# Bismarrck/tensoralloy

Hardware: AMD Instinct MI355X
Metric: atom-steps/sec (energy+forces), 4000-atom Ni rcut=6.5 A (higher is better)
Workload: dtype f64

## Files before the change

tensoralloy_amd/csrc/ta_api.hip:

```cpp
#include <hip/hip_runtime.h>

#include <algorithm>
#include <chrono>
#include <climits>
#include <cmath>
#include <cstdio>
#include <cstdlib>
#include <cstring>
#include <stdexcept>
#include <string>
#include <vector>

#include "ta_device.h"
#include "ta_internal.h"
#include "ta_md.h"

namespace ta {
size_t mlp_scratch_doubles(const MlpDev &mlp);
void launch_mlp_impl(const MlpDev &mlp, int activation, int ndim, const int32_t *atoms, int n_atoms,
                     const DeviceBatch &b, double *scratch, hipStream_t s, MlpLaunchInfo *info = nullptr);
size_t mlp_all_scratch_doubles(const MlpDev *mlps_host, int nel, const int32_t *elem_start);
size_t td_scratch_doubles(const MlpDev *nets, int nel, int K, const int32_t *elem_start);
void launch_td_all(const MlpDev *nets_dev, const MlpDev *nets_host, int nel, int K, int act_h, int act,
                   int sommerfeld, int ndim, const DeviceBatch &b, const double *T, double *u_atom,
// ... 1974 lines not shown
  if (h->kind != TA_MODEL_SF_MLP || !h->sf.angular)
    return fail(h, TA_ERR_INVALID, "only symmetry-function models with angular terms have triples");
  return guarded(h, [&]() {
    compute_impl(h, TA_WANT_ENERGY, false, nullptr);
    h->nl_stats.ensure(8);
    hipStream_t s = h->stream;
    HIP_CHECK(hipMemsetAsync(h->nl_stats.ptr, 0, sizeof(unsigned long long), s));
    const int64_t N = h->db.n_atoms;
    if (N)
      hipLaunchKernelGGL(count_triples_kernel, dim3((unsigned)((N * 64 + 255) / 256)), dim3(256), 0, s, h->db,
                         h->sf.acut * h->sf.acut, h->sf.eps, h->nl_stats.ptr, 1);
    HIP_CHECK(hipGetLastError());
    unsigned long long v = 0;
    HIP_CHECK(hipMemcpyAsync(&v, h->nl_stats.ptr, sizeof(v), hipMemcpyDeviceToHost, s));
    HIP_CHECK(hipStreamSynchronize(s));
    *n_owned = (int64_t)v;
  });
}

int ta_set_triangles(ta_handle h, int on) {
  if (!h) return TA_ERR_INVALID;
  h->triangles = on != 0;
  return TA_OK;
}

int ta_backward_variant(ta_handle h, int32_t *variant) {
  if (!h || !variant) return fail(h, TA_ERR_INVALID, "null argument");
  *variant = h->last_bwd_variant;
  return TA_OK;
}

int ta_mlp_launch_info(ta_handle h, int64_t *info) {
  if (!h || !info) return fail(h, TA_ERR_INVALID, "null argument");
  const ta::MlpLaunchInfo &m = h->last_mlp_launch;
  info[0] = m.family;
  info[1] = m.threads;
  info[2] = m.lh;
  info[3] = m.nt;
  info[4] = m.grid_x;
  info[5] = m.grid_y;
  info[6] = m.lds_bytes;
  info[7] = m.da;
  return TA_OK;
}

int ta_triangle_owner(int64_t n, const int32_t *abc, int32_t *owner) {
  if (n < 0 || (n > 0 && (!abc || !owner))) return TA_ERR_INVALID;
  for (int64_t t = 0; t < n; ++t) {
    int32_t a = abc[3 * t], b = abc[3 * t + 1], c = abc[3 * t + 2];
    if (a > b) std::swap(a, b);
    if (b > c) std::swap(b, c);
    if (a > b) std::swap(a, b);
    const int32_t sorted[3] = {a, b, c};
    owner[t] = (a == b || b == c) ? -1 : sorted[ta::triangle_owner_rank((uint32_t)a + (uint32_t)b + (uint32_t)c)];
  }
  return TA_OK;
}

int ta_measure_hbm_copy(ta_handle h, int64_t bytes, int32_t reps, double *gbs) {
  if (!h || !gbs || bytes < 16 || reps < 1) return fail(h, TA_ERR_INVALID, "bad argument");
  return guarded(h, [&]() {
    const size_t n = (size_t)bytes / 16;
    double2 *src = nullptr, *dst = nullptr;
    HIP_CHECK(hipMalloc((void **)&src, n * 16));
    if (hipMalloc((void **)&dst, n * 16) != hipSuccess) {
      (void)hipFree(src);
      throw std::bad_alloc();
    }
    hipStream_t s = h->stream;
    hipEvent_t e0, e1;
    HIP_CHECK(hipEventCreate(&e0));
    HIP_CHECK(hipEventCreate(&e1));
    HIP_CHECK(hipMemsetAsync(src, 0, n * 16, s));
    static const int per_cu = std::getenv("TA_COPY_WG_PER_CU") ? std::atoi(std::getenv("TA_COPY_WG_PER_CU")) : 8;
    const unsigned blocks = (unsigned)std::min<size_t>((n + 255) / 256, (size_t)256 * std::max(1, per_cu));
    static const int only = std::getenv("TA_COPY_MODE") ? std::atoi(std::getenv("TA_COPY_MODE")) : -1;
    double best = 0.0;
    for (int mode = 0; mode < 3; ++mode) {
      if (only >= 0 && mode != only) continue;
      auto one = [&]() {
        if (mode == 1) (void)hipMemcpyAsync(dst, src, n * 16, hipMemcpyDeviceToDevice, s);
        else if (mode == 2) hipLaunchKernelGGL(hbm_copy_nt_kernel, dim3(blocks), dim3(256), 0, s, src, dst, n);
        else hipLaunchKernelGGL(hbm_copy_kernel, dim3(blocks), dim3(256), 0, s, src, dst, n);
      };
      for (int k = 0; k < 2; ++k) one();
      HIP_CHECK(hipEventRecord(e0, s));
      for (int k = 0; k < reps; ++k) one();
      HIP_CHECK(hipEventRecord(e1, s));
      HIP_CHECK(hipEventSynchronize(e1));
      float ms = 0.f;
      HIP_CHECK(hipEventElapsedTime(&ms, e0, e1));
      if (ms > 0.f) best = std::max(best, 2.0 * (double)(n * 16) * reps / (ms * 1e-3) / 1e9);
    }
    (void)hipEventDestroy(e0);
    (void)hipEventDestroy(e1);
    (void)hipFree(src);
    (void)hipFree(dst);
    *gbs = best;
  });
}

int ta_set_stream(ta_handle h, void *stream) {
  if (!h) return TA_ERR_INVALID;
  return guarded(h, [&]() {
    HIP_CHECK(hipStreamSynchronize(h->stream));
    h->upload_pending = false;
    h->stream = stream ? (hipStream_t)stream : h->own_stream;
// ... 835 lines not shown
```

tensoralloy_amd/csrc/ta_device.h:

```cpp
#pragma once
#include <hip/hip_runtime.h>

#include <cstdint>

#include "tensoralloy_amd.h"

namespace ta {

constexpr int kMaxRadial = 64;
constexpr int kMaxElements = 8;
constexpr int kMaxBetaSlots = 3;
constexpr int kRecDoubles = 8;
constexpr int kMaxLayers = 8;
constexpr int kCapMin = 192;
constexpr int kCapMax = 1024;
constexpr int kMaxCentersPerBlock = 16;
constexpr int kMaxHd = 24;

struct SFParams {
  double rcut, acut;
  double inv_rc2, inv_ac2;
  double two_inv_ac2;
  double eps;
  double ang_scale;
// ... 20 lines not shown
  int chan[8];
  int safe_pow;
  int n_hd;
  double hd[kMaxHd];
};

struct DeviceBatch {
  int64_t n_atoms = 0, n_pairs = 0;
  int n_frames = 0, nnl_max = 0;
  double *pos = nullptr;
  double *cells = nullptr;
  int32_t *species = nullptr;
  int32_t *frame_of_atom = nullptr;
  int32_t *atom_start = nullptr;
  int32_t *pair_start = nullptr;
  int32_t *pair_stop = nullptr;
  int32_t *seg_start = nullptr;
  int32_t *pair_i = nullptr, *pair_j = nullptr, *pair_shift = nullptr, *pair_rev = nullptr;
  const int32_t *slot_q = nullptr, *rev_super = nullptr, *rev_map = nullptr;
  int32_t *blk_center = nullptr;
  int n_blk = 0;
  int blk_groups = 0;
  const int32_t *n_blk_dev = nullptr;
  int cap = kCapMin;
  int32_t *elem_atoms = nullptr;
  int32_t elem_start[kMaxElements + 1] = {0};

  double *rec = nullptr;
  double *rec4 = nullptr;
  double *part4 = nullptr;
  unsigned long long *masks = nullptr;
  uint32_t *job_word = nullptr;
  int32_t *job_count = nullptr;
  int job_stride = 0;
  uint32_t *job_word_own = nullptr;
  int32_t *job_count_own = nullptr;
  double *G = nullptr;
  double *dEdG = nullptr;
  double *eatom = nullptr;
  double *g = nullptr;
  double *forces = nullptr;
  double *wat = nullptr;
  double *fown = nullptr;
  int own_sums = 0;
#ifdef TA_PHASE_STAMPS
  unsigned long long *stamps = nullptr;
#endif
  double *bpart = nullptr;
  double *energy = nullptr;
  double *virial = nullptr;
  double *batch_energy = nullptr;
};

__host__ __device__ inline int triangle_owner_rank(uint32_t index_sum) {
#ifdef __HIP_DEVICE_COMPILE__
  const uint32_t h = __umul24(index_sum, 0x9E3779u);
#else
  const uint32_t h = index_sum * 0x9E3779u;
#endif
  return (int)(((h & 0xFFFFFFu) * 3u) >> 24);
}
__host__ __device__ inline bool owns_triangle(int32_t i, int32_t j, int32_t k) {
  return triangle_owner_rank((uint32_t)i + (uint32_t)j + (uint32_t)k) == (j < i ? 1 : 0) + (k < i ? 1 : 0);
}

#ifdef __HIPCC__
__device__ __forceinline__ int pair_stop_of(const DeviceBatch &b, int64_t i) {
  return b.pair_stop ? b.pair_stop[i] : b.pair_start[i + 1];
}
#endif

#ifdef __HIPCC__
__device__ __forceinline__ int pair_rev_of(const DeviceBatch &b, int q) {
  return b.slot_q ? b.rev_map[b.rev_super[b.slot_q[q]]] : b.pair_rev[q];
}
__device__ __forceinline__ const double2 *pair_geom(const DeviceBatch &b, size_t q) {
  return reinterpret_cast<const double2 *>(b.rec4 ? b.rec4 + 4 * q : b.rec + kRecDoubles * q);
}
#endif

struct MlpLayerDev {
  int k, n;
  int kp, np;
  double *w;
  double *wt;
  double *b;
  int act;
  int res;
};
struct MlpDev {
  int n_layers = 0;
  MlpLayerDev layer[kMaxLayers];
  double *xlo = nullptr, *xhi = nullptr;
  int max_np = 0, max_kp = 0;
};

struct MlpLaunchInfo {
  int family = 0;
  int threads = 0;
  int lh = 0;
  int nt = 0;
  int grid_x = 0, grid_y = 0;
  long long lds_bytes = 0;
  int da = 0;
};

void launch_pair_geometry(const SFParams &sf, const DeviceBatch &b, hipStream_t s);
void launch_g4_forward(const SFParams &sf, const AngChunk &ch, int nb, int ng, int nz,
                       const DeviceBatch &b, hipStream_t s);
void launch_descriptor_reduce(const SFParams &sf, const DeviceBatch &b, hipStream_t s);
void launch_mlp(const SFParams &sf, const MlpDev &mlp, int activation, int element,
                const DeviceBatch &b, hipStream_t s);
void launch_backward(const SFParams &sf, const AngChunk &ch, int nb, int ng, int nz,
                     bool first, bool radial_only, const DeviceBatch &b, hipStream_t s);
void launch_force_gather(const SFParams &sf, const DeviceBatch &b, hipStream_t s);
void launch_frame_reduce(const DeviceBatch &b, bool want_virial, double *mirror, int64_t n_tail, hipStream_t s);
// ... 68 lines not shown
```

tensoralloy_amd/csrc/ta_kernels_v2.hip:

```cpp
#include <hip/hip_runtime.h>

#include <cstdio>
#include <cstdlib>
#include <stdexcept>
#include <type_traits>

#include "ta_device.h"
#include "ta_math.h"
#include "ta_reduce.h"

namespace ta {
namespace {

constexpr int kBlock = 256;
constexpr int kNF = 8;
constexpr int kNFf = 7;
constexpr int kSegW = 6;
constexpr int kOwnCtl = 60 + 2 * kMaxCentersPerBlock * kSegW;
constexpr int kJobCtlBytes = (kOwnCtl + 40) * 4;
__host__ __device__ inline int v2_pcols(int cap, int nspec) {
  return nspec >= 1 ? cap / 4 + kMaxCentersPerBlock * nspec : cap;
}
constexpr int kRingPad = 64;
constexpr int kRTab = 8;

#ifdef TA_LDS_PROBE
__device__ __forceinline__ bool kProbe(int flags, int bit) { return (flags >> bit) & 1; }
#else
__device__ __forceinline__ constexpr bool kProbe(int, int) { return false; }
#endif

#ifdef TA_PHASE_STAMPS
#define TA_STAMP(b, kernel, k)                                                                          \
  do {                                                                                                  \
    if ((b).stamps && threadIdx.x == 0)                                                                 \
      (b).stamps[((size_t)(kernel) * gridDim.x + blockIdx.x) * 8 + (k)] = __builtin_amdgcn_s_memrealtime(); \
  } while (0)
#else
#define TA_STAMP(b, kernel, k) do {} while (0)
#endif

__device__ __forceinline__ int angular_term2(int s1, int s2, int nel) {
  int a = s1 < s2 ? s1 : s2, b = s1 < s2 ? s2 : s1;
  return a * nel - (a * (a - 1)) / 2 + (b - a);
}
__device__ __forceinline__ int radial_term2(int center, int other) {
  return other == center ? 0 : (other < center ? other + 1 : other);
}

struct Fields {
  double2 *zr, *xy, *ih, *gs;
  double *sp1;
  float *xf, *yf, *zf;
};

__device__ __forceinline__ Fields carve(double *lds, int cap, bool forward = false) {
  Fields f;
  f.zr = reinterpret_cast<double2 *>(lds);
  f.xy = f.zr + cap;
  f.ih = f.xy + cap;
  f.gs = forward ? nullptr : f.ih + cap;
  f.sp1 = forward ? reinterpret_cast<double *>(f.ih + cap) : nullptr;
  f.xf = forward ? reinterpret_cast<float *>(f.sp1 + cap) : nullptr;
  f.yf = forward ? f.xf + (2 * cap + kRingPad) : nullptr;
  f.zf = forward ? f.yf + (2 * cap + kRingPad) : nullptr;
  return f;
}

template <int HD>
__device__ __forceinline__ void hd_eval(const SFParams &sf, const AngChunk &ch, double beta,
                                        double u, double &h, double &dh) {
  if constexpr (HD > 0) {
    double p = ch.hd[HD - 1], d = 0.0;
#pragma unroll
    for (int k = HD - 2; k >= 0; --k) {
      d = fma(d, u, p);
      p = fma(p, u, ch.hd[k]);
    }
    h = p;
    dh = d;
  } else {
    double fd, dfd;
    cutoff_u(sf.cutoff, u, fd, dfd);
    const double ed = ta_exp(-beta * u);
    h = ed * fd;
    dh = ed * (dfd - beta * fd);
  }
}
template <int HD>
__device__ __forceinline__ double hd_value(const SFParams &sf, const AngChunk &ch, double beta,
                                           double u) {
  if constexpr (HD > 0) {
    double p = ch.hd[HD - 1];
#pragma unroll
    for (int k = HD - 2; k >= 0; --k) p = fma(p, u, ch.hd[k]);
    return p;
  } else {
    return ta_exp(-beta * u) * cutoff_u_value(sf.cutoff, u);
  }
}

template <int HD>
__device__ __forceinline__ void stage(const SFParams &sf, const AngChunk &ch, double beta, const DeviceBatch &b,
                                      const Fields &f, int s0, int M, int geom = 0, bool forward = false,
                                      int *jidx = nullptr) {
  for (int item = threadIdx.x; item < M; item += blockDim.x) {
    double2 v0, v1, v2;
    if (geom) {
      const int64_t p = (int64_t)s0 + item;
      const int i = b.pair_i[p], j = b.pair_j[p];
      const double *h = b.cells + 9 * (size_t)b.frame_of_atom[i];
      const double sx = (double)b.pair_shift[3 * p], sy = (double)b.pair_shift[3 * p + 1],
                   sz = (double)b.pair_shift[3 * p + 2];
      const double *ri = b.pos + 3 * (size_t)i, *rj = b.pos + 3 * (size_t)j;
      const double dx = (rj[0] - ri[0]) + (sx * h[0] + sy * h[3] + sz * h[6]);
      const double dy = (rj[1] - ri[1]) + (sx * h[1] + sy * h[4] + sz * h[7]);
      const double dz = (rj[2] - ri[2]) + (sx * h[2] + sy * h[5] + sz * h[8]);
      const double r2 = dx * dx + dy * dy + dz * dz + sf.eps;
      v0 = make_double2(dx, dy);
      v1 = make_double2(dz, r2);
      v2 = make_double2(1.0 / sqrt(r2), 0.0);
      if (b.rec4) {
        double2 *dst = reinterpret_cast<double2 *>(b.rec4 + 4 * (size_t)p);
        dst[0] = v0;
        dst[1] = v1;
      } else {
        double2 *dst = reinterpret_cast<double2 *>(b.rec + kRecDoubles * (size_t)p);
        dst[0] = v0;
        dst[1] = v1;
        dst[2] = v2;
        dst[3] = make_double2(0.0, 0.0);
      }
    } else if (b.rec4) {
      const double2 *src = reinterpret_cast<const double2 *>(b.rec4 + 4 * (size_t)(s0 + item));
      v0 = src[0];
      v1 = src[1];
      v2 = make_double2(1.0 / sqrt(v1.y), 0.0);
    } else {
      const double2 *src = reinterpret_cast<const double2 *>(b.rec + kRecDoubles * (size_t)(s0 + item));
      v0 = src[0];
      v1 = src[1];
      v2 = src[2];
    }
    f.xy[item] = v0;
    f.zr[item] = v1;
    if (forward) {
      const int ci = b.pair_i[s0 + item];
      const int cbase = b.pair_start[ci] - s0, cn = pair_stop_of(b, ci) - b.pair_start[ci];
      const int k0 = 2 * cbase + (item - cbase);
      f.xf[k0] = f.xf[k0 + cn] = (float)v0.x;
      f.yf[k0] = f.yf[k0 + cn] = (float)v0.y;
      f.zf[k0] = f.zf[k0 + cn] = (float)v1.x;
    }
    const double u = v1.y * sf.inv_ac2;
    double H = 0.0, L = 0.0;
    if (u < 1.0) {
      if (forward) {
        H = hd_value<HD>(sf, ch, beta, u);
      } else {
        double dH;
        hd_eval<HD>(sf, ch, beta, u, H, dH);
        L = (H != 0.0) ? sf.two_inv_ac2 * dH / H : 0.0;
      }
    }
    f.ih[item] = make_double2(v2.x, H);
    if (jidx) jidx[item] = b.pair_j[s0 + item];
    else if (forward) f.sp1[item] = (double)b.species[b.pair_j[s0 + item]];
    else f.gs[item] = make_double2(L, (double)b.species[b.pair_j[s0 + item]]);
  }
  __syncthreads();
}

__device__ __forceinline__ unsigned long long partner_mask(const SFParams &sf, const Fields &f,
                                                           int base, int n, int a, int sc, int smax) {
  const int ring = 2 * base + a;
  const float ax = f.xf[ring], ay = f.yf[ring], az = f.zf[ring];
  const float lim = (float)(sf.acut * sf.acut) * 1.0001f;
  unsigned long long mask = 0ull;
  const int count = smax - sc + 1;
  typedef float f32x2 __attribute__((ext_vector_type(2)));
  const f32x2 ax2 = {ax, ax}, ay2 = {ay, ay}, az2 = {az, az};
  for (int g = 0; g < 4 && 16 * g < count; ++g) {
    const float *px = f.xf + ring + sc + 16 * g, *py = f.yf + ring + sc + 16 * g,
                *pz = f.zf + ring + sc + 16 * g;
    unsigned m = 0u;
#pragma unroll
    for (int k = 14; k >= 0; k -= 2) {
      const f32x2 vx = {px[k], px[k + 1]}, vy = {py[k], py[k + 1]}, vz = {pz[k], pz[k + 1]};
      const f32x2 ex = vx - ax2, ey = vy - ay2, ez = vz - az2;
      const f32x2 d2 = __builtin_elementwise_fma(ex, ex, __builtin_elementwise_fma(ey, ey, ez * ez));
      const float dhi = d2.y, dlo = d2.x;
      asm("v_cmp_lt_f32 vcc, %1, %2\n\tv_addc_co_u32 %0, vcc, %0, %0, vcc" : "+v"(m) : "v"(dhi), "v"(lim) : "vcc");
      asm("v_cmp_lt_f32 vcc, %1, %2\n\tv_addc_co_u32 %0, vcc, %0, %0, vcc" : "+v"(m) : "v"(dlo), "v"(lim) : "vcc");
    }
    mask |= (unsigned long long)m << (16 * g);
  }
  if (count < 64) mask &= (1ull << count) - 1ull;
  const int half = n >> 1;
  if (!(n & 1) && a >= half && half >= sc && half < sc + 64) mask &= ~(1ull << (half - sc));
  return mask;
}

__device__ __forceinline__ void deal_by_popcount(const Fields &f, int cap, int M, int &item,
                                                 unsigned long long &mask) {
  int *hist = reinterpret_cast<int *>(f.xf);
  int *start = hist + 66;
  unsigned long long *pmask = reinterpret_cast<unsigned long long *>(hist + 132);
  int *pitem = reinterpret_cast<int *>(pmask + cap);
  const int tid = threadIdx.x;
  const bool active = tid < M;
  __syncthreads();
  if (tid < 66) hist[tid] = 0;
  __syncthreads();
  const int bucket = 64 - (active ? __popcll(mask) : 0);
  int rank = 0;
  if (active) rank = atomicAdd(&hist[bucket], 1);
  __syncthreads();
  if (tid < 65) {
    int s = 0;
// ... 68 lines not shown
  }
  const int n = j.start[16];
  __syncthreads();
  return n;
}

__device__ __forceinline__ int job_slot(int r, int tid, int T) { return r * T + ((r & 1) ? T - 1 - tid : tid); }

__device__ __forceinline__ void make_owned_jobs(int *hist, int *start, const uint32_t word[4], const unsigned own[4],
                                                uint32_t *out, int32_t *count) {
  const int tid = threadIdx.x;
  int cnt[4], rank[4] = {0, 0, 0, 0};
#pragma unroll
  for (int r = 0; r < 4; ++r) {
    cnt[r] = __popc(own[r]);
    if (cnt[r]) rank[r] = atomicAdd(&hist[16 - cnt[r]], 1);
  }
  __syncthreads();
  if (tid < 64) {
    const int v = tid < 16 ? hist[tid] : 0;
    int incl = v;
#pragma unroll
    for (int off = 1; off < 16; off <<= 1) {
      const int u = __shfl_up(incl, off);
      if (tid >= off) incl += u;
    }
    if (tid < 16) start[tid] = incl - v;
    if (tid == 15) *count = incl;
  }
  __syncthreads();
#pragma unroll
  for (int r = 0; r < 4; ++r)
    if (cnt[r]) out[start[16 - cnt[r]] + rank[r]] = (word[r] & 0xffffu) | (own[r] << 16);
}

template <int NG, int NZ>
__device__ __forceinline__ void defz_coeffs(const AngChunk &ch, const double *wsrc, double pc[5]) {
  double p0 = 0.0, p1 = 0.0, p2 = 0.0, p3 = 0.0, p4 = 0.0;
#pragma unroll
  for (int ig = 0; ig < NG; ++ig) {
    const double g1 = ch.gamma[ig], g2 = g1 * g1;
    const double w1 = wsrc[ch.chan[ig * NZ]] * ch.kz[0], w4 = wsrc[ch.chan[ig * NZ + 1]] * ch.kz[1];
    p0 += w1 + w4;
    p1 += g1 * (w1 + 4.0 * w4);
    p2 += 6.0 * g2 * w4;
    p3 += 4.0 * g2 * g1 * w4;
    p4 += g2 * g2 * w4;
  }
  pc[0] = p0;
  pc[1] = 0.5 * p1;
  pc[2] = 0.25 * p2;
  pc[3] = 0.125 * p3;
  pc[4] = 0.0625 * p4;
}

__device__ __forceinline__ double rsqrt_f64(double x) {
  double y = __builtin_amdgcn_rsq(x);
  const double hx = 0.5 * x;
  y = fma(y, fma(-hx * y, y, 0.5), y);
  y = fma(y, fma(-hx * y, y, 0.5), y);
  return y;
}

__device__ __forceinline__ void reduce_radial_from_lds(const SFParams &sf, const DeviceBatch &b,
                                                       const Fields &f, int c0, int c1, int s0) {
  const int nel = sf.n_elements;
  const int w = threadIdx.x >> 6, l = threadIdx.x & 63, nwaves = blockDim.x >> 6;
  bool no_shift = true;
  for (int c = 0; c < sf.n_rad; ++c) no_shift = no_shift && sf.omega[c] == 0.0;
  for (int64_t i = c0 + w; i < c1; i += nwaves) {
    const int sA = b.species[i];
    const int32_t *seg = b.seg_start + (size_t)i * (nel + 1);
    double *Gi = b.G + (size_t)i * sf.ndim;
    for (int sb = 0; sb < nel; ++sb) {
      const int tr = radial_term2(sA, sb);
      const int q0 = seg[sb] - s0, q1 = seg[sb + 1] - s0;
      for (int cc = 0; cc < sf.n_rad; cc += 4) {
        double acc[4] = {0.0, 0.0, 0.0, 0.0};
        for (int q = q0 + l; q < q1; q += 64) {
          const double r2 = f.zr[q].y;
          const double u = r2 * sf.inv_rc2;
          const double fc = (u < 1.0) ? cutoff_u_value(sf.cutoff, u) : 0.0;
          if (no_shift) {
#pragma unroll
            for (int k = 0; k < 4; ++k) {
              const int c = (cc + k < sf.n_rad) ? cc + k : cc;
              acc[k] += ta_exp(-sf.eta[c] * u) * fc;
            }
          } else {
            const double r = sqrt(r2);
#pragma unroll
            for (int k = 0; k < 4; ++k) {
              const int c = (cc + k < sf.n_rad) ? cc + k : cc;
              const double dr = r - sf.omega[c];
              acc[k] += ta_exp(-sf.eta[c] * dr * dr * sf.inv_rc2) * fc;
            }
          }
        }
#pragma unroll
        for (int k = 0; k < 4; ++k) {
          const double v = wave_sum(acc[k]);
          if (l == 0 && cc + k < sf.n_rad) Gi[tr * sf.n_rad + cc + k] = v;
        }
      }
    }
  }
// ... 89 lines not shown
        const int *ss = sslot + ci * kSegW;
        const double *colA = P + (size_t)(sa * kGZ + gz) * v2_pcols(cap, NSPEC);
        for (int q = ss[sb] + l; q < ss[sb + 1]; q += 16) v += colA[q];
        if (sa != sb) {
          const double *colB = P + (size_t)(sb * kGZ + gz) * v2_pcols(cap, NSPEC);
          for (int q = ss[sa] + l; q < ss[sa + 1]; q += 16) v += colB[q];
        }
        v = row16_sum(v);
        if (l == 0) Gi[sf.n_radial_dim + term * sf.n_ang + ch.chan[gz]] = v * sf.ang_scale;
      }
    }
  }
}

__device__ __forceinline__ void stagger(int flags) {
  const int n = (flags >> 8) & 0xff;
  if (n && ((blockIdx.x >> ((flags >> 16) & 31)) & 1))
    for (int k = 0; k < n; ++k) __builtin_amdgcn_s_sleep(127);
}

template <int NSPEC, int NG, int NZ, int HD, bool DEFZ, int CAP, int WPE = (DEFZ && NSPEC <= 2 ? 5 : 0)>
__global__ __launch_bounds__(kBlock)
    __attribute__((amdgpu_waves_per_eu(WPE > 0 ? WPE : 1, 8))) void g4_forward_v2_kernel(SFParams sf, AngChunk ch,
                                                               DeviceBatch b, int flags) {
  static_assert(!DEFZ || NZ == 2, "DEFZ needs the two-zeta grid");
  const int kCap = CAP > 0 ? CAP : b.cap;
  const int geom = flags & 1;
  if (b.n_blk_dev && (int)blockIdx.x >= *b.n_blk_dev) return;
  stagger(flags);
  extern __shared__ double lds[];
  const Fields f = carve(lds, kCap, true);
  const int slot = b.blk_groups > 0 ? 16 * ((int)blockIdx.x % b.blk_groups) + (int)blockIdx.x / b.blk_groups
                                    : (int)blockIdx.x;
  const int c0 = b.blk_center[slot], c1 = b.blk_center[slot + 1];
  if (c0 >= c1) return;
  const int s0 = b.pair_start[c0];
  const int M = pair_stop_of(b, c1 - 1) - s0;
  const double beta = ch.beta[0];
  if (b.job_count) {
    char *raw = reinterpret_cast<char *>(lds);
    int *cnt = reinterpret_cast<int *>(raw + v2_counter_offset(kCap));
    if (threadIdx.x < 40) cnt[threadIdx.x] = 0;
    else if (threadIdx.x < 40 + 17 && (int)threadIdx.x - 40 <= c1 - c0)
      cnt[threadIdx.x] = ((int)threadIdx.x - 40 < c1 - c0 ? b.pair_start[c0 + threadIdx.x - 40] : s0 + M) - s0;
    else if (threadIdx.x >= 64 && (int)threadIdx.x - 64 < (c1 - c0) * (NSPEC + 1)) {
      const int k = ((int)threadIdx.x - 64) / (NSPEC + 1), sg = ((int)threadIdx.x - 64) % (NSPEC + 1);
      cnt[60 + k * kSegW + sg] = b.seg_start[(size_t)(c0 + k) * (NSPEC + 1) + sg] - s0;
    }
    if (NSPEC == 1 && b.job_word_own && threadIdx.x < 20) cnt[kOwnCtl + threadIdx.x] = 0;
    double *P0 = reinterpret_cast<double *>(raw + v2_counter_offset(kCap) + kJobCtlBytes);
    for (int k = threadIdx.x; k < NSPEC * NG * NZ * v2_pcols(kCap, NSPEC); k += blockDim.x) P0[k] = 0.0;
  }
  int *jidx = (NSPEC == 1 && b.job_word_own && b.job_count) ? reinterpret_cast<int *>(f.sp1) : nullptr;
  TA_STAMP(b, 0, 0);
  stage<HD>(sf, ch, beta, b, f, s0, M, geom, true, jidx);
  TA_STAMP(b, 0, 1);
  if (b.job_count && threadIdx.x == 0) {
    int *ctl = reinterpret_cast<int *>(reinterpret_cast<char *>(lds) + v2_counter_offset(kCap));
    const int *segl = ctl + 60;
    int *sslot = ctl + 60 + kMaxCentersPerBlock * kSegW;
    int acc = 0;
    for (int k = 0; k < c1 - c0; ++k)
      for (int sg = 0; sg <= NSPEC; ++sg) {
        sslot[k * kSegW + sg] = acc;
        if (sg < NSPEC) acc += (segl[k * kSegW + sg + 1] - segl[k * kSegW + sg] + 3) >> 2;
      }
  }

  auto run_item = [&](int item, bool have_mask, unsigned long long mask0, double *out, double *pacc, auto is_job) {
    constexpr bool kJob = decltype(is_job)::value;
    const int64_t p = (int64_t)s0 + item;
    int base, n;
    int pslot = item;
    unsigned own = 0u;
    int kbit = 0;
    uint32_t sij = 0u;
    int ic = 0, rij = 0;
    if constexpr (kJob) {
      const int *cstart = reinterpret_cast<const int *>(reinterpret_cast<const char *>(lds) + v2_counter_offset(kCap)) + 40;
      const int ci = job_centre((uint32_t)mask0);
      if (NSPEC == 1 && jidx) {
        ic = c0 + ci;
        const int j = jidx[item];
        sij = (uint32_t)ic + (uint32_t)j;
        rij = j < ic ? 1 : 0;
      }
      base = cstart[ci];
      n = cstart[ci + 1] - base;
      {
        const int *segl = cstart + 20, *sslot = segl + kMaxCentersPerBlock * kSegW;
        const int sg = NSPEC == 1 ? 0 : (int)f.sp1[item];
        pslot = sslot[ci * kSegW + sg] + ((item - segl[ci * kSegW + sg]) >> 2);
      }
    } else {
      const int i = b.pair_i[p];
      base = b.pair_start[i] - s0;
      n = pair_stop_of(b, i) - b.pair_start[i];
    }
    const int a = item - base;
    const double2 axy = f.xy[item], azr = f.zr[item], aih = f.ih[item];
    const double ax = axy.x, ay = axy.y, az = azr.x;
    const double ra2 = azr.y, inv_ra = aih.x, Ha = aih.y;

    double acc[NSPEC][NG][NZ];
#pragma unroll
    for (int sp = 0; sp < NSPEC; ++sp)
#pragma unroll
      for (int ig = 0; ig < NG; ++ig)
#pragma unroll
        for (int iz = 0; iz < NZ; ++iz) acc[sp][ig][iz] = 0.0;
    double mom[NSPEC][5];
#pragma unroll
    for (int sp = 0; sp < NSPEC; ++sp)
#pragma unroll
      for (int k = 0; k < 5; ++k) mom[sp][k] = 0.0;

    auto triple = [&](int bl) {
        bl = (int)min((unsigned)bl, (unsigned)bl - (unsigned)n);
        const int q = kProbe(flags, 30) ? (int)threadIdx.x : base + bl;
        const double2 bxy = f.xy[q], bzr = f.zr[q];
        const double ex = bxy.x - ax, ey = bxy.y - ay, ez = bzr.x - az;
        const double d2 = fma(ex, ex, fma(ey, ey, fma(ez, ez, sf.eps)));
        const double u = kProbe(flags, 30) ? 0.5 : d2 * sf.inv_ac2;
        if (!(u < 1.0)) return;
        if constexpr (kJob && NSPEC == 1) {
          if (jidx) {
            const int kk = jidx[q];
            own |= (triangle_owner_rank(sij + (uint32_t)kk) == rij + (kk < ic ? 1 : 0) ? 1u : 0u) << kbit;
          }
        }
        const double2 bih = f.ih[kProbe(flags, 29) ? (int)threadIdx.x : q];
        const double cth = (ra2 + bzr.y - d2) * 0.5 * inv_ra * bih.x;
        const double common = Ha * bih.y * hd_value<HD>(sf, ch, beta, u);
        const int sb = NSPEC == 1 ? 0 : (int)f.sp1[q];
        if constexpr (DEFZ) {
          const double c2 = cth * cth;
          const double t1 = common * cth, t2 = common * c2, t3 = t1 * c2, t4 = t2 * c2;
#pragma unroll
          for (int sp = 0; sp < NSPEC; ++sp) {
            const bool on = NSPEC == 1 || sb == sp;
            mom[sp][0] += on ? common : 0.0;
            mom[sp][1] += on ? t1 : 0.0;
            mom[sp][2] += on ? t2 : 0.0;
            mom[sp][3] += on ? t3 : 0.0;
            mom[sp][4] += on ? t4 : 0.0;
          }
        } else {
#pragma unroll
          for (int ig = 0; ig < NG; ++ig) {
            const double basev = fma(ch.gamma[ig], cth, 1.0);
#pragma unroll
            for (int iz = 0; iz < NZ; ++iz) {
              double pw;
              if (ch.zeta_int[iz] > 0)
                pw = pow_int_m1(basev, ch.zeta_int[iz]) * basev;
              else
                pw = safe_pow_value(ch.safe_pow, basev, ch.zeta[iz]);
              const double v = pw * common;
#pragma unroll
              for (int sp = 0; sp < NSPEC; ++sp)
                acc[sp][ig][iz] += (NSPEC == 1 || sb == sp) ? v : 0.0;
            }
          }
        }
    };
    if constexpr (kJob) {
      const uint32_t jw = (uint32_t)mask0;
      unsigned m = (flags & (1 << 24)) ? 0u : jw >> 16;
      const int k0 = a + 1 + 16 * (int)((jw >> 8) & 3u);
      while (m) {
        const int k = __ffs((int)m) - 1;
        m &= m - 1;
        kbit = k;
        triple(k0 + k);
      }
    } else {
    const int smax = (Ha != 0.0) ? n / 2 : 0;
    for (int sc = 1; sc <= smax; sc += 64) {
      unsigned long long mask;
      if (have_mask) {
        mask = (flags & (1 << 24)) ? 0ull : mask0;
      } else {
        mask = partner_mask(sf, f, base, n, a, sc, smax);
        if (b.masks) b.masks[(size_t)(sc >> 6) * b.n_pairs + p] = mask;
      }
      while (mask) {
        const int k = __ffsll((long long)mask) - 1;
        mask &= mask - 1;
        triple(a + sc + k);
      }
    }
    }
    if constexpr (DEFZ) {
#pragma unroll
      for (int sp = 0; sp < NSPEC; ++sp)
#pragma unroll
        for (int ig = 0; ig < NG; ++ig) {
          const double g1 = ch.gamma[ig], g2 = g1 * g1;
          acc[sp][ig][0] = fma(g1, mom[sp][1], mom[sp][0]);
          acc[sp][ig][1] = fma(g2 * g2, mom[sp][4], fma(4.0 * g2 * g1, mom[sp][3],
                               fma(6.0 * g2, mom[sp][2], fma(4.0 * g1, mom[sp][1], mom[sp][0]))));
        }
    }
#pragma unroll
    for (int sp = 0; sp < NSPEC; ++sp)
#pragma unroll
      for (int ig = 0; ig < NG; ++ig)
#pragma unroll
        for (int iz = 0; iz < NZ; ++iz) {
          const int c = ch.chan[ig * NZ + iz];
          const double v = acc[sp][ig][iz] * ch.kz[iz];
          if (pacc) {
            if (v != 0.0) atomicAdd(&pacc[(size_t)((sp * NG + ig) * NZ + iz) * v2_pcols(kCap, NSPEC) + pslot], v);
          } else if (out)
            out[(sp * NG + ig) * NZ + iz] = v;
          else
            b.part4[(size_t)(sp * sf.n_ang + c) * b.n_pairs + p] = v;
        }
    return own;
  };

  int item = threadIdx.x;
  const bool active = item < M;
  int n_own = 0;
  if (active) {
    const int i = b.pair_i[s0 + item];
    n_own = pair_stop_of(b, i) - b.pair_start[i];
  }
  const bool one_pass = M <= (int)blockDim.x && !__syncthreads_or(active && (n_own >> 1) > 64);
  if (one_pass) {
    unsigned long long mask = 0ull;
    if (active) {
      const int64_t p = (int64_t)s0 + item;
      const int i = b.pair_i[p];
      const int base = b.pair_start[i] - s0;
      const int smax = (f.ih[item].y != 0.0) ? n_own / 2 : 0;
      if (smax > 0 && !(flags & (1 << 25))) mask = partner_mask(sf, f, base, n_own, item - base, 1, smax);
      if (b.masks && !b.job_count) b.masks[p] = mask;
    }
    TA_STAMP(b, 0, 2);
    if (b.job_count) {
      char *raw = reinterpret_cast<char *>(lds);
      JobLists jl = job_lists(f);
      jl.hist = reinterpret_cast<int *>(raw + v2_counter_offset(kCap));
      jl.start = jl.hist + 20;
      double *P = reinterpret_cast<double *>(raw + v2_counter_offset(kCap) + kJobCtlBytes);
      const int n_jobs = make_jobs(jl, active, item, active ? b.pair_i[s0 + item] - c0 : 0, mask);
      TA_STAMP(b, 0, 3);
      const size_t jbase = (size_t)blockIdx.x * b.job_stride;
      if (threadIdx.x == 0) b.job_count[blockIdx.x] = n_jobs;
      for (int slot = threadIdx.x; slot < n_jobs; slot += blockDim.x) b.job_word[jbase + slot] = jl.word[slot];
      TA_STAMP(b, 0, 4);
      uint32_t swept[4] = {0u, 0u, 0u, 0u};
      unsigned owned[4] = {0u, 0u, 0u, 0u};
      if (!(flags & (1 << 27)))
        for (int r = 0; r * (int)blockDim.x < n_jobs; ++r) {
          const int slot = job_slot(r, threadIdx.x, blockDim.x);
          if (slot < n_jobs) {
            const uint32_t jw = jl.word[slot];
            const unsigned o = run_item(job_item(jw), true, jw, nullptr, P, std::true_type{});
            if (r < 4) {
              swept[r] = jw;
              owned[r] = o;
            }
          }
        }
      if (jidx)
        make_owned_jobs(jl.hist + kOwnCtl, jl.hist + kOwnCtl + 20, swept, owned, b.job_word_own + jbase,
                        b.job_count_own + blockIdx.x);
      __syncthreads();
      TA_STAMP(b, 0, 5);
      if (flags & 4) {
        assemble_flat<NSPEC, NG, NZ>(sf, ch, b, f, P, jl.hist + 60 + kMaxCentersPerBlock * kSegW, c0, c1, s0, item, active,
                                     (flags & (1 << 26)) != 0, kCap);
        TA_STAMP(b, 0, 6);
        return;
      }
      if (active) {
        const int64_t p = (int64_t)s0 + threadIdx.x;
        const int ci = b.pair_i[p] - c0, sg = NSPEC == 1 ? 0 : (int)f.sp1[threadIdx.x];
        const int *segl = jl.hist + 60, *sslot = segl + kMaxCentersPerBlock * kSegW;
        const int rel = (int)threadIdx.x - segl[ci * kSegW + sg];
        const int pidx = sslot[ci * kSegW + sg] + (rel >> 2);
        const bool holds = (rel & 3) == 0;
#pragma unroll
        for (int sp = 0; sp < NSPEC; ++sp)
#pragma unroll
          for (int gz = 0; gz < NG * NZ; ++gz)
            b.part4[(size_t)(sp * sf.n_ang + ch.chan[gz]) * b.n_pairs + p] =
                holds ? P[(size_t)(sp * NG * NZ + gz) * v2_pcols(kCap, NSPEC) + pidx] : 0.0;
      }
    } else {
    deal_by_popcount(f, kCap, M, item, mask);
    constexpr int kLocal = NSPEC * NG * NZ;
    constexpr int kGZ = NG * NZ;
    constexpr int kSpPerPass = 8 / kGZ;
    if (flags & 4) {
      double mine[kLocal];
#pragma unroll
      for (int k = 0; k < kLocal; ++k) mine[k] = 0.0;
      if (active) run_item(item, true, mask, mine, nullptr, std::false_type{});
      __syncthreads();
      double *red = reinterpret_cast<double *>(f.xy);
#pragma unroll
      for (int sp_lo = 0; sp_lo < NSPEC; sp_lo += kSpPerPass) {
        const int sp_hi = sp_lo + kSpPerPass < NSPEC ? sp_lo + kSpPerPass : NSPEC;
        if (active) {
#pragma unroll
          for (int k = 0; k < kSpPerPass * kGZ; ++k)
            if (sp_lo * kGZ + k < kLocal) red[(size_t)k * kCap + item] = mine[sp_lo * kGZ + k];
        }
        __syncthreads();
        if (sp_lo == 0) reduce_radial_from_lds(sf, b, f, c0, c1, s0);
        reduce_angular_from_lds<NSPEC, NG, NZ>(sf, ch, b, red, kCap, c0, c1, s0, sp_lo, sp_hi);
        __syncthreads();
      }
      return;
    }
    if (active) run_item(item, true, mask, nullptr, nullptr, std::false_type{});
    }
  } else {
    if (b.job_count && threadIdx.x == 0) b.job_count[blockIdx.x] = -1;
    if (jidx && threadIdx.x == 0) b.job_count_own[blockIdx.x] = -1;
    for (int it = threadIdx.x; it < M; it += blockDim.x) run_item(it, false, 0ull, nullptr, nullptr, std::false_type{});
  }

  if (flags & 2) {
    __syncthreads();
    const int ncent = c1 - c0;
    const int nwaves = blockDim.x >> 6;
    if (ncent <= nwaves) {
      const int w = threadIdx.x >> 6, l = threadIdx.x & 63;
      const bool act = w < ncent;
      const int64_t i = c0 + (act ? w : 0);
      atom_descriptors<64>(sf, b, i, l, act, [&](int c, double v) { b.G[(size_t)i * sf.ndim + c] = v; });
    } else {
      const int row = threadIdx.x >> 4, l = threadIdx.x & 15, nrows = blockDim.x >> 4;
      for (int k0 = 0; k0 < ncent; k0 += nrows) {
        const bool act = k0 + row < ncent;
        const int64_t i = c0 + (act ? k0 + row : 0);
        atom_descriptors<16>(sf, b, i, l, act, [&](int c, double v) { b.G[(size_t)i * sf.ndim + c] = v; });
      }
    }
  }
}

template <int NSPEC, int NG, int NZ, int HD, bool DEFZ, int CAP, int WPE = (DEFZ ? (NSPEC <= 2 ? 5 : 4) : 0),
          bool TRI = false>
__global__ __launch_bounds__(kBlock)
    __attribute__((amdgpu_waves_per_eu(WPE > 0 ? WPE : 1, 8))) void backward_v2_kernel(SFParams sf, AngChunk ch,
                                                             DeviceBatch b, int flags) {
  static_assert(!DEFZ || NZ == 2, "DEFZ needs the two-zeta grid");
  static_assert(!TRI || (NSPEC == 1 && DEFZ && HD > 0), "the triangle build is one-element, default grid, Hd series");
  const int first = flags & 1;
  if (b.n_blk_dev && (int)blockIdx.x >= *b.n_blk_dev) return;
  stagger(flags);
  extern __shared__ double lds[];
  const int kCap = CAP > 0 ? CAP : b.cap;
  const Fields f = carve(lds, kCap);
  double *gacc = lds + kNF * kCap + kCap / 8;
  const int slot = b.blk_groups > 0 ? 16 * ((int)blockIdx.x % b.blk_groups) + (int)blockIdx.x / b.blk_groups
                                    : (int)blockIdx.x;
  const int c0 = b.blk_center[slot], c1 = b.blk_center[slot + 1];
  if (c0 >= c1) return;
  const int s0 = b.pair_start[c0];
  const int M = pair_stop_of(b, c1 - 1) - s0;
  const double beta = ch.beta[0];
  for (int k = threadIdx.x; k < 3 * kCap; k += blockDim.x) gacc[k] = 0.0;
  int *cstart = reinterpret_cast<int *>(gacc) - 20;
  if ((int)threadIdx.x <= c1 - c0 && threadIdx.x < 17)
    cstart[threadIdx.x] = ((int)threadIdx.x < c1 - c0 ? b.pair_start[c0 + threadIdx.x] : s0 + M) - s0;
  double *pctab = gacc + 3 * kCap;
  if constexpr (DEFZ && NSPEC == 1) {
    const int k = (int)blockDim.x - 1 - (int)threadIdx.x;
    if (k < c1 - c0) {
      const double *wsrc = b.dEdG + (size_t)(c0 + k) * sf.ndim + sf.n_radial_dim;
// ... 45 lines not shown

  auto run_tri = [&](int item, bool have_mask, unsigned long long mask0, auto is_job) {
    constexpr bool kJob = decltype(is_job)::value;
    const int64_t p = (int64_t)s0 + item;
    int i, base, n;
    if constexpr (kJob) {
      const int ci = job_centre((uint32_t)mask0);
      i = c0 + ci;
      base = cstart[ci];
      n = cstart[ci + 1] - base;
    } else {
      i = b.pair_i[p];
      base = b.pair_start[i] - s0;
      n = pair_stop_of(b, i) - b.pair_start[i];
    }
    const int a = item - base;
    const double2 axy = f.xy[item], azr = f.zr[item], aih = f.ih[item], ags = f.gs[item];
    const double ax = axy.x, ay = axy.y, az = azr.x;
    const double A = azr.y, inv_ra = aih.x, Ha = aih.y, La = ags.x;
    const double inv_A = inv_ra * inv_ra;
    double pi_[5], pj_[5];
#pragma unroll
    for (int k = 0; k < 5; ++k) pi_[k] = pctab[5 * (i - c0) + k];
    {
      const double2 p01 = pn01[item], p23 = pn23[item];
      pj_[0] = p01.x;
      pj_[1] = p01.y;
      pj_[2] = p23.x;
      pj_[3] = p23.y;
      pj_[4] = pn4[item];
    }
    const int ja = kJob ? 0 : b.pair_j[p];
    double csum = 0.0, gx = 0.0, gy = 0.0, gz = 0.0;
    auto tri = [&](int bl) {
      bl = (int)min((unsigned)bl, (unsigned)bl - (unsigned)n);
      const int q = base + bl;
      if constexpr (!kJob) {
        if (!owns_triangle(i, ja, b.pair_j[s0 + q])) return;
      }
      const double2 bxy = f.xy[q], bzr = f.zr[q];
      const double bx = bxy.x, by = bxy.y, bz = bzr.x;
      const double ex = bx - ax, ey = by - ay, ez = bz - az;
      const double D = fma(ex, ex, fma(ey, ey, fma(ez, ez, sf.eps)));
      const double u = D * sf.inv_ac2;
      if (!(u < 1.0)) return;
      const double2 bih = f.ih[q], bgs = f.gs[q], p01 = pn01[q], p23 = pn23[q];
      const double pk4 = pn4[q];
      const double B = bzr.y, inv_rb = bih.x, Hb = bih.y, Lb = bgs.x;
      double Hd, dHd;
      hd_eval<HD>(sf, ch, beta, u, Hd, dHd);
      const double inv_d = rsqrt_f64(D);
      const double inv_ab = inv_ra * inv_rb, inv_ad = inv_ra * inv_d, inv_bd = inv_rb * inv_d;
      const double wi = (A + B - D) * inv_ab, wj = (A + D - B) * inv_ad, wk = (B + D - A) * inv_bd;
      const double Si = fma(fma(fma(fma(pi_[4], wi, pi_[3]), wi, pi_[2]), wi, pi_[1]), wi, pi_[0]);
      const double Pi = fma(fma(fma(4.0 * pi_[4], wi, 3.0 * pi_[3]), wi, 2.0 * pi_[2]), wi, pi_[1]);
      const double Sj = fma(fma(fma(fma(pj_[4], wj, pj_[3]), wj, pj_[2]), wj, pj_[1]), wj, pj_[0]);
      const double Pj = fma(fma(fma(4.0 * pj_[4], wj, 3.0 * pj_[3]), wj, 2.0 * pj_[2]), wj, pj_[1]);
      const double Sk = fma(fma(fma(fma(pk4, wk, p23.y), wk, p23.x), wk, p01.y), wk, p01.x);
      const double Pk = fma(fma(fma(4.0 * pk4, wk, 3.0 * p23.y), wk, 2.0 * p23.x), wk, p01.y);
      const double HH = Ha * Hb, T = HH * Hd;
      const double sum = Si + Sj + Sk;
      const double TS = T * sum;
      const double X = (sum * HH) * (sf.two_inv_ac2 * dHd);
      const double Yi = Pi * T, Yj = Pj * T, Yk = Pk * T;
      const double Ywi = Yi * wi, Ywj = Yj * wj, Ywk = Yk * wk;
      const double inv_D = inv_d * inv_d;
      const double ZD = (Ywj + Ywk) * inv_D;
      const double Yjd = Yj * inv_ad, Ykd = Yk * inv_bd;
      const double ca = fma(TS, La, fma(-(Ywi + Ywj), inv_A, fma(4.0, Yjd, X - ZD)));
      const double cb = fma(TS, Lb, fma(-(Ywi + Ywk), inv_rb * inv_rb, fma(4.0, Ykd, X - ZD)));
      const double Q = fma(2.0, fma(Yi, inv_ab, -(Yjd + Ykd)), ZD - X);
      csum += ca;
      gx = fma(Q, bx, gx);
      gy = fma(Q, by, gy);
      gz = fma(Q, bz, gz);
      atomicAdd(&gacc[q], fma(cb, bx, Q * ax));
      atomicAdd(&gacc[kCap + q], fma(cb, by, Q * ay));
      atomicAdd(&gacc[2 * kCap + q], fma(cb, bz, Q * az));
    };
    if constexpr (kJob) {
      const uint32_t jw = (uint32_t)mask0;
      unsigned m = (flags & (1 << 24)) ? 0u : jw >> 16;
      const int k0 = a + 1 + 16 * (int)((jw >> 8) & 3u);
      while (m) {
        const int k = __ffs((int)m) - 1;
        m &= m - 1;
        tri(k0 + k);
      }
    } else {
      const int smax = (Ha != 0.0) ? n / 2 : 0;
      for (int sc = 1; sc <= smax; sc += 64) {
        unsigned long long mask = have_mask ? mask0 : b.masks[(size_t)(sc >> 6) * b.n_pairs + p];
        if (flags & (1 << 24)) mask = 0ull;
        while (mask) {
          const int k = __ffsll((long long)mask) - 1;
          mask &= mask - 1;
          tri(a + sc + k);
        }
      }
    }
    atomicAdd(&gacc[item], fma(csum, ax, gx));
    atomicAdd(&gacc[kCap + item], fma(csum, ay, gy));
    atomicAdd(&gacc[2 * kCap + item], fma(csum, az, gz));
  };

  auto run_item = [&](int item, bool have_mask, unsigned long long mask0, auto is_job) {
    constexpr bool kJob = decltype(is_job)::value;
    const int64_t p = (int64_t)s0 + item;
    int i, base, n;
    if constexpr (kJob) {
      const int ci = job_centre((uint32_t)mask0);
      i = c0 + ci;
// ... 29 lines not shown
    double pc[NSPEC][5];
    if constexpr (kTable) {
      const double *src = pctab + 5 * (i - c0);
#pragma unroll
      for (int k = 0; k < 5; ++k) pc[0][k] = src[k];
    } else if constexpr (DEFZ) {
#pragma unroll
      for (int sp = 0; sp < NSPEC; ++sp) {
#pragma unroll
        for (int k = 0; k < 5; ++k) pc[sp][k] = 0.0;
#pragma unroll
        for (int ig = 0; ig < NG; ++ig) {
          const double g1 = ch.gamma[ig], g2 = g1 * g1;
          const double w1 = w_[sp][ig][0], w4 = w_[sp][ig][1];
          pc[sp][0] += w1 + w4;
          pc[sp][1] += 0.5 * g1 * (w1 + 4.0 * w4);
          pc[sp][2] += 0.25 * 6.0 * g2 * w4;
          pc[sp][3] += 0.125 * 4.0 * g2 * g1 * w4;
          pc[sp][4] += 0.0625 * g2 * g2 * w4;
        }
      }
    }
    double csum = 0.0, gx = 0.0, gy = 0.0, gz = 0.0;
    auto triple = [&](int bl) {
        bl = (int)min((unsigned)bl, (unsigned)bl - (unsigned)n);
        const int q = kProbe(flags, 30) ? (int)threadIdx.x : base + bl;
        const double2 bxy = f.xy[q], bzr = f.zr[q];
        const double bx = bxy.x, by = bxy.y, bz = bzr.x;
        const double ex = bx - ax, ey = by - ay, ez = bz - az;
        const double d2 = fma(ex, ex, fma(ey, ey, fma(ez, ez, sf.eps)));
        const double u = kProbe(flags, 30) ? 0.5 : d2 * sf.inv_ac2;
        if (!(u < 1.0)) return;
        const int q2 = kProbe(flags, 29) ? (int)threadIdx.x : q;
        const double2 bih = f.ih[q2], bgs = f.gs[q2];
        const double inv_rb = bih.x, Hb = bih.y, Lb = bgs.x;
        const int sb = NSPEC == 1 ? 0 : (int)bgs.y;
        const double inv_ab = inv_ra * inv_rb;
        const double w = (ra2 + bzr.y - d2) * inv_ab;
        double Hd, dHd;
        hd_eval<HD>(sf, ch, beta, u, Hd, dHd);
        const double Hd2 = sf.two_inv_ac2 * dHd;
        double S0 = 0.0, Yc, Y;
        const double HH = Ha * Hb, T = HH * Hd;
        if constexpr (DEFZ) {
          double p0 = pc[0][0], p1 = pc[0][1], p2 = pc[0][2], p3 = pc[0][3], p4 = pc[0][4];
#pragma unroll
          for (int sp = 1; sp < NSPEC; ++sp) {
            p0 = (sb == sp) ? pc[sp][0] : p0;
            p1 = (sb == sp) ? pc[sp][1] : p1;
            p2 = (sb == sp) ? pc[sp][2] : p2;
            p3 = (sb == sp) ? pc[sp][3] : p3;
            p4 = (sb == sp) ? pc[sp][4] : p4;
          }
          S0 = fma(fma(fma(fma(p4, w, p3), w, p2), w, p1), w, p0);
          const double S1w = fma(fma(fma(4.0 * p4, w, 3.0 * p3), w, 2.0 * p2), w, p1);
          const double Z = S1w * T;
          Yc = Z * w;
          Y = Z + Z;
        } else {
          const double cth = 0.5 * w;
          double S1 = 0.0;
#pragma unroll
          for (int ig = 0; ig < NG; ++ig) {
            const double basev = fma(ch.gamma[ig], cth, 1.0);
#pragma unroll
            for (int iz = 0; iz < NZ; ++iz) {
              double ws = w_[0][ig][iz], wds = wd[0][ig][iz];
#pragma unroll
              for (int sp = 1; sp < NSPEC; ++sp) {
                ws = (sb == sp) ? w_[sp][ig][iz] : ws;
                wds = (sb == sp) ? wd[sp][ig][iz] : wds;
              }
              double pm1;
              if (ch.zeta_int[iz] > 0)
                pm1 = pow_int_m1(basev, ch.zeta_int[iz]);
              else
                pm1 = safe_pow_grad(ch.safe_pow, basev, ch.zeta[iz] - 1.0);
              S0 = fma(ws, pm1 * basev, S0);
              S1 = fma(wds, pm1, S1);
            }
          }
          Y = S1 * T;
          Yc = Y * cth;
        }
        const double S0T = S0 * T;
        const double X = (S0 * HH) * Hd2;
        const double ca = fma(S0T, La, fma(-Yc, inv_ra2, X));
        const double cb = fma(S0T, Lb, fma(-Yc, inv_rb * inv_rb, X));
        const double Q = fma(Y, inv_ab, -X);
        csum += ca;
        gx = fma(Q, bx, gx);
        gy = fma(Q, by, gy);
        gz = fma(Q, bz, gz);
        const int q3 = kProbe(flags, 28) ? (int)threadIdx.x : q;
        atomicAdd(&gacc[q3], fma(cb, bx, Q * ax));
        atomicAdd(&gacc[kCap + q3], fma(cb, by, Q * ay));
        atomicAdd(&gacc[2 * kCap + q3], fma(cb, bz, Q * az));
    };
    if constexpr (kJob) {
      const uint32_t jw = (uint32_t)mask0;
      unsigned m = (flags & (1 << 24)) ? 0u : jw >> 16;
      const int k0 = a + 1 + 16 * (int)((jw >> 8) & 3u);
      while (m) {
        const int k = __ffs((int)m) - 1;
        m &= m - 1;
        triple(k0 + k);
      }
    } else {
// ... 276 lines not shown
```

Before: 36.95 million.

## Use per-index residue tokens and LUT for triangle ownership; Horner derivative tweaks

Changes the triangle ownership hash from a hash of the index sum to a sum of per-index residues mod 3. This lets the staged pair slot hold a precomputed token (residue plus a j<i flag), and the inner loop decides ownership with one LDS token read and a 24-bit lookup-table bit test. It also rewrites the polynomial-plus-derivative evaluations as a single interleaved Horner pass, hoists Ha and 0.5*inv_ra out of the inner loop, and pins eps/inv_ac2 in scalar registers. The ownership assignment changes (different owners per triangle), which must stay consistent between host and device, and the polynomial rewrite slightly changes rounding.

```diff
diff --git a/tensoralloy_amd/csrc/ta_api.hip b/tensoralloy_amd/csrc/ta_api.hip
--- a/tensoralloy_amd/csrc/ta_api.hip
+++ b/tensoralloy_amd/csrc/ta_api.hip
@@ -2050,7 +2050,7 @@
     if (b > c) std::swap(b, c);
     if (a > b) std::swap(a, b);
     const int32_t sorted[3] = {a, b, c};
-    owner[t] = (a == b || b == c) ? -1 : sorted[ta::triangle_owner_rank((uint32_t)a + (uint32_t)b + (uint32_t)c)];
+    owner[t] = (a == b || b == c) ? -1 : sorted[ta::triangle_owner_rank((uint32_t)a, (uint32_t)b, (uint32_t)c)];
   }
   return TA_OK;
 }
diff --git a/tensoralloy_amd/csrc/ta_device.h b/tensoralloy_amd/csrc/ta_device.h
--- a/tensoralloy_amd/csrc/ta_device.h
+++ b/tensoralloy_amd/csrc/ta_device.h
@@ -96,16 +96,30 @@
   double *batch_energy = nullptr;
 };
 
-__host__ __device__ inline int triangle_owner_rank(uint32_t index_sum) {
+__host__ __device__ inline uint32_t owner_residue(uint32_t x) {
 #ifdef __HIP_DEVICE_COMPILE__
-  const uint32_t h = __umul24(index_sum, 0x9E3779u);
+  const uint32_t h = __umul24(x, 0x9E3779u);
 #else
-  const uint32_t h = index_sum * 0x9E3779u;
-#endif
-  return (int)(((h & 0xFFFFFFu) * 3u) >> 24);
-}
+  const uint32_t h = x * 0x9E3779u;
+#endif
+  return ((h & 0xFFFFFFu) * 3u) >> 24;
+}
+__host__ __device__ inline int triangle_owner_rank(uint32_t a, uint32_t b, uint32_t c) {
+  return (int)((owner_residue(a) + owner_residue(b) + owner_residue(c)) % 3u);
+}
+__host__ __device__ inline uint32_t owner_token(int32_t j, int32_t i) {
+  return owner_residue((uint32_t)j) + (j < i ? 8u : 0u);
+}
+constexpr uint32_t owner_lut() {
+  uint32_t lut = 0u;
+  for (uint32_t c = 0; c < 24u; ++c)
+    if ((c & 7u) < 7u && (c & 7u) % 3u == (c >> 3)) lut |= 1u << c;
+  return lut;
+}
+constexpr uint32_t kOwnerLut = owner_lut();
+static_assert(kOwnerLut == 0x241249u, "ownership table");
 __host__ __device__ inline bool owns_triangle(int32_t i, int32_t j, int32_t k) {
-  return triangle_owner_rank((uint32_t)i + (uint32_t)j + (uint32_t)k) == (j < i ? 1 : 0) + (k < i ? 1 : 0);
+  return (kOwnerLut >> (owner_residue((uint32_t)i) + owner_token(j, i) + owner_token(k, i))) & 1u;
 }
 
 #ifdef __HIPCC__
diff --git a/tensoralloy_amd/csrc/ta_kernels_v2.hip b/tensoralloy_amd/csrc/ta_kernels_v2.hip
--- a/tensoralloy_amd/csrc/ta_kernels_v2.hip
+++ b/tensoralloy_amd/csrc/ta_kernels_v2.hip
@@ -71,9 +71,9 @@
 __device__ __forceinline__ void hd_eval(const SFParams &sf, const AngChunk &ch, double beta,
                                         double u, double &h, double &dh) {
   if constexpr (HD > 0) {
-    double p = ch.hd[HD - 1], d = 0.0;
-#pragma unroll
-    for (int k = HD - 2; k >= 0; --k) {
+    double d = ch.hd[HD - 1], p = fma(d, u, ch.hd[HD - 2]);
+#pragma unroll
+    for (int k = HD - 3; k >= 0; --k) {
       d = fma(d, u, p);
       p = fma(p, u, ch.hd[k]);
     }
@@ -164,7 +164,7 @@
       }
     }
     f.ih[item] = make_double2(v2.x, H);
-    if (jidx) jidx[item] = b.pair_j[s0 + item];
+    if (jidx) jidx[item] = (int)owner_token(b.pair_j[s0 + item], b.pair_i[s0 + item]);
     else if (forward) f.sp1[item] = (double)b.species[b.pair_j[s0 + item]];
     else f.gs[item] = make_double2(L, (double)b.species[b.pair_j[s0 + item]]);
   }
@@ -339,6 +339,17 @@
   pc[2] = 0.25 * p2;
   pc[3] = 0.125 * p3;
   pc[4] = 0.0625 * p4;
+}
+
+__device__ __forceinline__ void poly4_eval(double p0, double p1, double p2, double p3, double p4, double w,
+                                           double &S, double &dS) {
+  double p = fma(p4, w, p3), d = fma(p4, w, p);
+  p = fma(p, w, p2);
+  d = fma(d, w, p);
+  p = fma(p, w, p1);
+  d = fma(d, w, p);
+  S = fma(p, w, p0);
+  dS = d;
 }
 
 __device__ __forceinline__ double rsqrt_f64(double x) {
@@ -534,6 +545,7 @@
     for (int k = threadIdx.x; k < NSPEC * NG * NZ * v2_pcols(kCap, NSPEC); k += blockDim.x) P0[k] = 0.0;
   }
   int *jidx = (NSPEC == 1 && b.job_word_own && b.job_count) ? reinterpret_cast<int *>(f.sp1) : nullptr;
+  const bool want_own = jidx != nullptr;
   TA_STAMP(b, 0, 0);
   stage<HD>(sf, ch, beta, b, f, s0, M, geom, true, jidx);
   TA_STAMP(b, 0, 1);
@@ -556,17 +568,13 @@
     int pslot = item;
     unsigned own = 0u;
     int kbit = 0;
-    uint32_t sij = 0u;
-    int ic = 0, rij = 0;
+    uint32_t tok_a = 0u;
+    typedef __attribute__((address_space(3))) const int lds_cint;
+    const uint32_t tok_base = (uint32_t)(uintptr_t)(lds_cint *)f.sp1;
     if constexpr (kJob) {
       const int *cstart = reinterpret_cast<const int *>(reinterpret_cast<const char *>(lds) + v2_counter_offset(kCap)) + 40;
       const int ci = job_centre((uint32_t)mask0);
-      if (NSPEC == 1 && jidx) {
-        ic = c0 + ci;
-        const int j = jidx[item];
-        sij = (uint32_t)ic + (uint32_t)j;
-        rij = j < ic ? 1 : 0;
-      }
+      if (NSPEC == 1 && jidx) tok_a = owner_residue((uint32_t)(c0 + ci)) + (uint32_t)jidx[item];
       base = cstart[ci];
       n = cstart[ci + 1] - base;
       {
@@ -583,6 +591,9 @@
     const double2 axy = f.xy[item], azr = f.zr[item], aih = f.ih[item];
     const double ax = axy.x, ay = axy.y, az = azr.x;
     const double ra2 = azr.y, inv_ra = aih.x, Ha = aih.y;
+    const double half_inv_ra = 0.5 * inv_ra;
+    double eps = sf.eps, inv_ac2 = sf.inv_ac2;
+    if constexpr (kJob) asm volatile("" : "+s"(eps), "+s"(inv_ac2));
 
     double acc[NSPEC][NG][NZ];
 #pragma unroll
@@ -602,18 +613,16 @@
         const int q = kProbe(flags, 30) ? (int)threadIdx.x : base + bl;
         const double2 bxy = f.xy[q], bzr = f.zr[q];
         const double ex = bxy.x - ax, ey = bxy.y - ay, ez = bzr.x - az;
-        const double d2 = fma(ex, ex, fma(ey, ey, fma(ez, ez, sf.eps)));
-        const double u = kProbe(flags, 30) ? 0.5 : d2 * sf.inv_ac2;
+        const double d2 = fma(ex, ex, fma(ey, ey, fma(ez, ez, eps)));
+        const double u = kProbe(flags, 30) ? 0.5 : d2 * inv_ac2;
         if (!(u < 1.0)) return;
         if constexpr (kJob && NSPEC == 1) {
-          if (jidx) {
-            const int kk = jidx[q];
-            own |= (triangle_owner_rank(sij + (uint32_t)kk) == rij + (kk < ic ? 1 : 0) ? 1u : 0u) << kbit;
-          }
+          const uint32_t tb = (uint32_t)*reinterpret_cast<lds_cint *>(tok_base + 4u * (uint32_t)q);
+          own |= ((kOwnerLut >> ((tok_a + tb) & 31u)) & 1u) << kbit;
         }
         const double2 bih = f.ih[kProbe(flags, 29) ? (int)threadIdx.x : q];
-        const double cth = (ra2 + bzr.y - d2) * 0.5 * inv_ra * bih.x;
-        const double common = Ha * bih.y * hd_value<HD>(sf, ch, beta, u);
+        const double cth = (ra2 + bzr.y - d2) * half_inv_ra * bih.x;
+        const double common = bih.y * hd_value<HD>(sf, ch, beta, u);
         const int sb = NSPEC == 1 ? 0 : (int)f.sp1[q];
         if constexpr (DEFZ) {
           const double c2 = cth * cth;
@@ -691,7 +700,7 @@
 #pragma unroll
         for (int iz = 0; iz < NZ; ++iz) {
           const int c = ch.chan[ig * NZ + iz];
-          const double v = acc[sp][ig][iz] * ch.kz[iz];
+          const double v = acc[sp][ig][iz] * (ch.kz[iz] * Ha);
           if (pacc) {
             if (v != 0.0) atomicAdd(&pacc[(size_t)((sp * NG + ig) * NZ + iz) * v2_pcols(kCap, NSPEC) + pslot], v);
           } else if (out)
@@ -747,7 +756,7 @@
             }
           }
         }
-      if (jidx)
+      if (want_own)
         make_owned_jobs(jl.hist + kOwnCtl, jl.hist + kOwnCtl + 20, swept, owned, b.job_word_own + jbase,
                         b.job_count_own + blockIdx.x);
       __syncthreads();
@@ -803,7 +812,7 @@
     }
   } else {
     if (b.job_count && threadIdx.x == 0) b.job_count[blockIdx.x] = -1;
-    if (jidx && threadIdx.x == 0) b.job_count_own[blockIdx.x] = -1;
+    if (want_own && threadIdx.x == 0) b.job_count_own[blockIdx.x] = -1;
     for (int it = threadIdx.x; it < M; it += blockDim.x) run_item(it, false, 0ull, nullptr, nullptr, std::false_type{});
   }
 
@@ -955,12 +964,19 @@
       const double inv_d = rsqrt_f64(D);
       const double inv_ab = inv_ra * inv_rb, inv_ad = inv_ra * inv_d, inv_bd = inv_rb * inv_d;
       const double wi = (A + B - D) * inv_ab, wj = (A + D - B) * inv_ad, wk = (B + D - A) * inv_bd;
-      const double Si = fma(fma(fma(fma(pi_[4], wi, pi_[3]), wi, pi_[2]), wi, pi_[1]), wi, pi_[0]);
-      const double Pi = fma(fma(fma(4.0 * pi_[4], wi, 3.0 * pi_[3]), wi, 2.0 * pi_[2]), wi, pi_[1]);
-      const double Sj = fma(fma(fma(fma(pj_[4], wj, pj_[3]), wj, pj_[2]), wj, pj_[1]), wj, pj_[0]);
-      const double Pj = fma(fma(fma(4.0 * pj_[4], wj, 3.0 * pj_[3]), wj, 2.0 * pj_[2]), wj, pj_[1]);
-      const double Sk = fma(fma(fma(fma(pk4, wk, p23.y), wk, p23.x), wk, p01.y), wk, p01.x);
-      const double Pk = fma(fma(fma(4.0 * pk4, wk, 3.0 * p23.y), wk, 2.0 * p23.x), wk, p01.y);
+      double Si, Pi, Sj, Pj, Sk, Pk;
+      if constexpr (kJob) {
+        poly4_eval(pi_[0], pi_[1], pi_[2], pi_[3], pi_[4], wi, Si, Pi);
+        poly4_eval(pj_[0], pj_[1], pj_[2], pj_[3], pj_[4], wj, Sj, Pj);
+        poly4_eval(p01.x, p01.y, p23.x, p23.y, pk4, wk, Sk, Pk);
+      } else {
+        Si = fma(fma(fma(fma(pi_[4], wi, pi_[3]), wi, pi_[2]), wi, pi_[1]), wi, pi_[0]);
+        Pi = fma(fma(fma(4.0 * pi_[4], wi, 3.0 * pi_[3]), wi, 2.0 * pi_[2]), wi, pi_[1]);
+        Sj = fma(fma(fma(fma(pj_[4], wj, pj_[3]), wj, pj_[2]), wj, pj_[1]), wj, pj_[0]);
+        Pj = fma(fma(fma(4.0 * pj_[4], wj, 3.0 * pj_[3]), wj, 2.0 * pj_[2]), wj, pj_[1]);
+        Sk = fma(fma(fma(fma(pk4, wk, p23.y), wk, p23.x), wk, p01.y), wk, p01.x);
+        Pk = fma(fma(fma(4.0 * pk4, wk, 3.0 * p23.y), wk, 2.0 * p23.x), wk, p01.y);
+      }
       const double HH = Ha * Hb, T = HH * Hd;
       const double sum = Si + Sj + Sk;
       const double TS = T * sum;
@@ -1096,8 +1112,8 @@
             p3 = (sb == sp) ? pc[sp][3] : p3;
             p4 = (sb == sp) ? pc[sp][4] : p4;
           }
-          S0 = fma(fma(fma(fma(p4, w, p3), w, p2), w, p1), w, p0);
-          const double S1w = fma(fma(fma(4.0 * p4, w, 3.0 * p3), w, 2.0 * p2), w, p1);
+          double S1w;
+          poly4_eval(p0, p1, p2, p3, p4, w, S0, S1w);
           const double Z = S1w * T;
           Yc = Z * w;
           Y = Z + Z;
```

Measured after the change: 37.32 million, median of 6. 1.0% higher.
